# hydradarpa/kalman-hydra

Measured on AMD Instinct MI355X. Metric: frames/sec (Brox flow + EKF update) at 1024^2, higher is better.
Workload: dtype f32 (flow, renders) / f64 (EKF sums and state)

## Files before the change

### kalman-hydra_amd/csrc/ekf.hip

```cpp
#include "hm_common.h"
#include "ekf_kernels.h"
#include "dense_kernels.h"
#include "chol_flow_kernels.h"
#include "project_kernels.h"
#include "predict_kernels.h"
#include "view_kernels.h"
#include "body_kernels.h"
#include "roi_kernels.h"
#include "smooth_kernels.h"
#include <algorithm>
#include <atomic>
#include <chrono>
#include <cmath>
#include <condition_variable>
#include <cstring>
#include <functional>
#include <mutex>
#include <set>
#include <thread>
#include <utility>
#include <vector>

struct Helper {
    std::thread th;
// ... 21 lines not shown
        }
    }
    void post(std::function<int()> f)
    {
        std::unique_lock<std::mutex> lk(m);
        if (!th.joinable()) th = std::thread([this] { run(); });
        job = std::move(f);
        posted = busy = true;
        cv.notify_all();
    }
    int wait()
    {
        std::unique_lock<std::mutex> lk(m);
        cv.wait(lk, [&] { return !busy; });
        const int r = rc;
        rc = HM_OK;
        return r;
    }
    void stop()
    {
        {
            std::unique_lock<std::mutex> lk(m);
            cv.wait(lk, [&] { return !busy; });
            quit = true;
            cv.notify_all();
        }
        if (th.joinable()) th.join();
    }
};

struct hm_ctx {
    int device, W, H, N, T, E, njobs;
    HmOwner own{1};
    Helper helper;
    bool helper_used = false;
    int tail_async = 1;
    double eps_Z, eps_J, eps_M;
    hipStream_t stream;
    int *d_tri, *d_star_off, *d_star_tri, *d_edges;
    int *d_nb_off = nullptr, *d_nb_u = nullptr, *d_nb_e = nullptr;
    float *d_uv;
    uint8_t *d_tex;
    std::vector<int> edges;
    uint8_t *d_yim, *d_ym;
    float *d_yfx, *d_yfy, *d_yfxm, *d_yfym;
    bool obs_owned = true;
    const uint8_t *o_yim, *o_ym;
    const float *o_yfx, *o_yfy;
    bool have_tex, have_obs, have_ref;
    Targets ref, P, Q;
    TriSetup *d_setup, *d_cfgs;
    int4 *d_ubox;
    int *d_tlist = nullptr, *d_tcount = nullptr;
    unsigned *d_tmask = nullptr;
    double *d_X, *d_out, *d_partial;
    uint8_t *d_im8, *d_m8;
    std::vector<double> X0;
    double *d_HTH;
    double *d_H, *d_Hz, *d_Hzc, *d_invW0, *d_Af[2], *d_T[2], *d_step, *d_Wtmp, *d_X0, *d_Xn, *d_Wprior, *d_gain, *d_Awork, *d_Lt[2];
    std::vector<double> upd_X0;
    int upd_last = -1, upd_prev = -1;
    double *d_Wres;
    double *pin;
    size_t pin_n;
    int *pin_scratch;
    std::vector<double> resv, tailv;
    int result_delay = 0;
    bool tail_pending = false;
    bool tail_valid = false;
    long long tail_ticket = 0;
    hipStream_t tail_stream = nullptr;
    const uint8_t *armed_mask = nullptr;
    std::vector<int> sp_h_off, sp_h_bar, sp_h_other;
    std::vector<double> sp_h_blk;
    std::vector<int32_t> sp_bars_cached;
    std::vector<int> tri;
    DPool pool;
    int *d_area;
    int *d_sp_off, *d_sp_bar, *d_sp_other;
    double *d_sp_blk;
    bool upd_open;
    bool prefactored;
    std::vector<double> h_partial;
    int red_blocks = 512;
    double *d_tpart = nullptr;
    std::vector<double> h_tpart;
    int ntiles = 0;
    int render_rows = RI_H;
    bool last_err_valid = false;
    double last_err[4] = {0, 0, 0, 0};
    std::vector<double> last_err_X;
    long long run_ticket;
    int vsplit = 5, esplit;
    bool pn_armed = false;
    void *pn_worker = nullptr;
    std::vector<int32_t> pn_bars;
    std::vector<double> pn_l0;
    double pn_par[4] = {0, 0, 0, 0};
    int pn_maxiter = 0;
    bool pq_armed = false;
    double pq_eps_F = 0.0;
    bool pq_valid = false;
    std::vector<double> pq_X, pq_l0;
    std::vector<int32_t> pq_bars;
    double pq_par[4] = {0, 0, 0, 0};
    hipStream_t stream3 = nullptr;
// ... 269 lines not shown
    h->eps_Z = eps_Z; h->eps_J = eps_J; h->eps_M = eps_M;
    h->tri.assign(tri, tri + (size_t)3 * T);
    for (const auto &e : eset) { h->edges.push_back(e.first); h->edges.push_back(e.second); }
    h->E = (int)eset.size();
    h->njobs = N + h->E;
    h->esplit = 2 * h->E > 1024 ? 1 : 2;
    const size_t n = (size_t)W * H;
    int rc = HM_OK;
    auto step = [&](int r) { if (rc == HM_OK) rc = r; };
    step(upload(h->own, &h->d_tri, tri, (size_t)3 * T));
    step(upload(h->own, &h->d_uv, uv, (size_t)2 * N));
    step(upload(h->own, &h->d_star_off, off.data(), off.size()));
    step(upload(h->own, &h->d_star_tri, flat.data(), flat.size()));
    step(upload(h->own, &h->d_edges, h->edges.data(), h->edges.size()));
    {
        std::vector<std::vector<std::pair<int, int>>> nb(N);
        for (int e = 0; e < h->E; e++) {
            const int a = h->edges[2 * e], b = h->edges[2 * e + 1];
            nb[a].push_back(std::make_pair(b, e));
            nb[b].push_back(std::make_pair(a, e));
        }
        std::vector<int> noff(N + 1, 0), nu, ne;
        for (int v = 0; v < N; v++) {
            std::sort(nb[v].begin(), nb[v].end());
            noff[v + 1] = noff[v] + (int)nb[v].size();
            for (const auto &q : nb[v]) { nu.push_back(q.first); ne.push_back(q.second); }
            if (rc == HM_OK && 4 * ((int)nb[v].size() + 1) > PREP_MAX_ENTRIES) {
                hm_set_error("hm_ctx_create: vertex %d has %d neighbours, limit %d", v, (int)nb[v].size(), PREP_MAX_ENTRIES / 4 - 1);
                rc = HM_ERR_ARG;
            }
        }
        step(upload(h->own, &h->d_nb_off, noff.data(), noff.size()));
        step(upload(h->own, &h->d_nb_u, nu.data(), nu.size()));
        step(upload(h->own, &h->d_nb_e, ne.data(), ne.size()));
    }
    hipError_t e = hipSuccess;
    auto dev = [&](auto **p, size_t bytes) { if (e == hipSuccess) e = h->own.alloc(p, bytes); };
    if (rc == HM_OK) {
        const char *pe = getenv("HYDRA_MI_EKF_PRIORITY");
        e = h->own.stream(&h->stream, !(pe && atoi(pe) == 0));
        dev(&h->d_tex, n);
        dev(&h->d_yim, n);
        dev(&h->d_ym, n);
        dev(&h->d_yfx, n * sizeof(float));
        dev(&h->d_yfy, n * sizeof(float));
        dev(&h->d_yfxm, n * sizeof(float));
        dev(&h->d_yfym, n * sizeof(float));
        dev(&h->d_setup, (size_t)T * sizeof(TriSetup));
        dev(&h->d_cfgs, (size_t)N * MEAS_NCFG * (EKF_MAX_STAR + 1) * sizeof(TriSetup));
        dev(&h->d_ubox, (size_t)N * UBOX_STRIDE * sizeof(int4));
        dev(&h->d_tmask, (size_t)N * TMASK_STRIDE * sizeof(unsigned));
        dev(&h->d_tlist, (size_t)N * TMASK_STRIDE * sizeof(int));
        dev(&h->d_tcount, (size_t)N * sizeof(int));
        dev(&h->d_X, (size_t)4 * N * sizeof(double));
        dev(&h->d_out, (size_t)h->njobs * MEAS_VSPLIT_MAX * MEAS_OUT * sizeof(double));
        dev(&h->d_partial, (size_t)h->red_blocks * 4 * sizeof(double));
        h->ntiles = hm_cdiv(W, RI_W) * hm_cdiv(H, 8);
        dev(&h->d_tpart, (size_t)h->ntiles * RI_NV * sizeof(double));
        dev(&h->d_im8, n);
        dev(&h->d_m8, n);
        const size_t n4 = (size_t)4 * N, nn = n4 * n4 * sizeof(double);
        dev(&h->d_H, nn);
        dev(&h->d_HTH, nn);
        if (e == hipSuccess) e = hipMemsetAsync(h->d_HTH, 0, nn, h->stream);
        dev(&h->d_invW0, nn);
        const size_t nn_aug = (size_t)(hm_cdiv((int)n4, DNB) * DNB + DNB) * n4 * sizeof(double);
        dev(&h->d_Af[0], nn_aug);
        dev(&h->d_Af[1], nn_aug);
        dev(&h->d_Awork, nn_aug);
        const size_t ld_bytes = (size_t)hm_cdiv((int)n4, DNB) * DNB * DNB * sizeof(double);
        dev(&h->d_T[0], nn);
        dev(&h->d_T[1], nn);
        dev(&h->d_step, n4 * sizeof(double));
        dev(&h->d_Lt[0], ld_bytes);
        dev(&h->d_Lt[1], ld_bytes);
        dev(&h->d_Wtmp, nn);
        dev(&h->d_flowP, 3 * ld_bytes);
        dev(&h->d_flowctl, 4 * sizeof(unsigned));
        if (e == hipSuccess) e = hipMemsetAsync(h->d_flowctl, 0, 4 * sizeof(unsigned), h->stream);
        dev(&h->d_Hz, n4 * sizeof(double));
        dev(&h->d_Hzc, n4 * 4 * sizeof(double));
        dev(&h->d_Wprior, nn);
        dev(&h->d_gain, n4 * 3 * sizeof(double));
        h->pin_n = 2 * (n4 + RES_HEAD + n4 * 4 + n4 * 3) + 2;
        if (e == hipSuccess) e = h->own.host_alloc(&h->pin, h->pin_n * sizeof(double), hipHostMallocCoherent);
        if (e == hipSuccess) memset(h->pin, 0, h->pin_n * sizeof(double));
        h->pin_scratch = (int *)(h->pin + h->pin_n - 2);
        h->resv.assign(n4 + RES_HEAD, 0.0);
        h->tailv.assign(n4 * 7, 0.0);
        dev(&h->d_X0, n4 * sizeof(double));
        dev(&h->pool.hdr, (size_t)4 * N * sizeof(int));
        dev(&h->pool.overflow, sizeof(int));
        dev(&h->d_area, (size_t)N * sizeof(int));
        h->pool.area = h->d_area;
        if (e == hipSuccess) e = pool_alloc(h, (long long)8 * W * H);
        dev(&h->d_Xn, n4 * sizeof(double));
        for (Targets *t : {&h->ref, &h->P, &h->Q})
            if (e == hipSuccess) e = alloc_targets(h->own, *t, n);
    }
    if (e != hipSuccess) {
        hm_set_error("hm_ctx_create: device allocation failed: %s", hipGetErrorString(e));
        step(HM_ERR_HIP);
    }
    if (rc != HM_OK) {
        ctx_free(h);
        return rc;
// ... 453 lines not shown
    rc = render_ids(h, h->X0.data(), h->ref, h->d_ids[0], true);
    if (rc == HM_OK) rc = render_ids(h, Xp.data(), h->P, h->d_ids[1], false);
    if (rc == HM_OK) rc = render_ids(h, Xq.data(), h->Q, h->d_ids[2], false);
    if (rc) return rc;
    MultiArgs a = {h->ref, h->P, h->Q, h->d_ids[0], h->d_ids[1], h->d_ids[2], obs_of(h, 0), h->W, h->d_lbox, h->d_lout};
    hipLaunchKernelGGL(k_j_multi, dim3(n_labels), dim3(RED_NT), 0, h->stream, a);
    HM_HIP(hipGetLastError());
    h->h_lout.resize((size_t)n_labels * 5);
    HM_HIP(hipMemcpyAsync(h->h_lout.data(), h->d_lout, (size_t)n_labels * 5 * sizeof(double), hipMemcpyDeviceToHost, h->stream));
    HM_HIP(hipStreamSynchronize(h->stream));
    for (int l = 0; l < n_labels; l++) {
        const double *s = h->h_lout.data() + 5 * l;
        const double c[4] = {s[0] / h->eps_Z, s[1] / h->eps_J, s[2] / h->eps_J, s[3] / h->eps_M};
        hsum[l] = ((c[0] + c[1]) + c[2]) + c[3];
        nz[l] = s[4];
        if (hcomp) for (int k = 0; k < 4; k++) hcomp[4 * l + k] = c[k];
    }
    return HM_OK;
}

extern "C" int hm_error(hm_ctx_t h, const double *X, int masked, double err[4], float *fx, float *fy)
{
    HM_ARG(h && X && err, "hm_error: NULL argument");
    HM_JOIN(h);
    NEED_TEX(h, "hm_error");
    NEED_OBS(h, "hm_error");
    HM_HIP(hipSetDevice(h->device));
    HM_HIP(hipMemcpyAsync(h->d_X, X, (size_t)4 * h->N * sizeof(double), hipMemcpyHostToDevice, h->stream));
    int rc = render_iter(h, h->d_X, h->P, true, masked, false, 2.0);
    if (rc) return rc;
    const int n = h->W * h->H;
    if (fx) HM_HIP(hipMemcpyAsync(fx, h->P.fx, (size_t)n * sizeof(float), hipMemcpyDeviceToHost, h->stream));
    if (fy) HM_HIP(hipMemcpyAsync(fy, h->P.fy, (size_t)n * sizeof(float), hipMemcpyDeviceToHost, h->stream));
    HM_HIP(hipMemcpyAsync(h->h_tpart.data(), h->d_tpart, (size_t)render_strips(h) * RI_NV * sizeof(double), hipMemcpyDeviceToHost, h->stream));
    HM_HIP(stream_wait(h->stream));
    double s6[RI_NV];
    hm_tile_partial_sums(h->h_tpart.data(), render_strips(h), s6);
    for (int k = 0; k < 4; k++) err[k] = s6[k];
    return HM_OK;
}

static int measure_dev(hm_ctx *h, const double *dX, bool ref_ready, double deltaX, int masked, bool regions_ready = false,
                       bool scatter = true)
{
    if (!ref_ready) {
        int rc = render_iter(h, dX, h->ref, false, masked, !regions_ready, deltaX);
        if (rc) return rc;
        regions_ready = true;
    }
    MeasureArgs a;
    measure_args(h, dX, deltaX, masked, a);
    if (!regions_ready) hipLaunchKernelGGL(k_star_regions, dim3(h->N), dim3(REGION_NT), 0, h->stream, a, h->d_area);
    hipLaunchKernelGGL(k_measure_vertex, dim3(h->N, h->vsplit), dim3(MEAS_NT), 0, h->stream, a,
                       (const TriSetup *)h->d_cfgs, (const int4 *)h->d_ubox, (const unsigned *)h->d_tmask);
    if (h->E > 0) hipLaunchKernelGGL(k_measure_edge, dim3(h->E, h->esplit), dim3(MEAS_NT), 0, h->stream, a);
    if (scatter) {
        ScatterArgs s = {h->d_out, h->d_edges, h->N, h->E, h->vsplit, h->esplit, h->eps_Z, h->eps_J, h->eps_M, deltaX, h->d_HTH, h->d_Hz, h->d_Hzc};
        hipLaunchKernelGGL(k_hth_scatter, dim3(hm_cdiv(h->njobs, 4)), dim3(256), 0, h->stream, s);
    }
    HM_HIP(hipGetLastError());
    return HM_OK;
}

static void measure_args(hm_ctx *h, const double *dX, double deltaX, int masked, MeasureArgs &a)
{
    a.m = Mesh{h->W, h->H, h->N, h->T, h->d_tri, h->d_uv, h->d_tex};
    a.topo = StarTopo{h->d_star_off, h->d_star_tri, h->d_edges, h->E};
    a.ref = h->ref;
    a.obs = obs_of(h, masked);
    a.X = dX;
    a.delta = deltaX;
    a.out = h->d_out;
    a.pool = h->pool;
    a.vsplit = h->vsplit;
    a.esplit = h->esplit;
    a.iZ = 1.0 / h->eps_Z; a.iJ = 1.0 / h->eps_J; a.iM = 1.0 / h->eps_M;
    a.cfgs = h->d_cfgs;
    a.ubox = h->d_ubox;
    a.tmask = h->d_tmask;
    a.tlist = h->d_tlist;
    a.tcount = h->d_tcount;
    a.tmask_stride = TMASK_STRIDE;
}

static int measure_on_device(hm_ctx *h, const double *X, double deltaX, int masked, bool scatter = true)
{
    HM_HIP(hipMemcpyAsync(h->d_X, X, (size_t)4 * h->N * sizeof(double), hipMemcpyHostToDevice, h->stream));
    h->X0.assign(X, X + 4 * h->N);
    h->have_ref = true;
    return measure_dev(h, h->d_X, false, deltaX, masked, false, scatter);
}

extern "C" int hm_measure(hm_ctx_t h, const double *X, double deltaX, int masked, double *Hz, double *Hzc, double *HTH)
{
    HM_ARG(h && X && Hz && HTH, "hm_measure: NULL argument");
    HM_JOIN(h);
    HM_ARG(deltaX > 0, "hm_measure: deltaX must be positive");
    NEED_TEX(h, "hm_measure");
    NEED_OBS(h, "hm_measure");
    HM_HIP(hipSetDevice(h->device));
    const size_t n4 = (size_t)4 * h->N;
    int *ovf = h->pin_scratch;
    for (int attempt = 0;; attempt++) {
        int rc = measure_on_device(h, X, deltaX, masked);
        if (rc) return rc;
        *ovf = 0;
        HM_HIP(hipMemcpyAsync(ovf, h->pool.overflow, sizeof(int), hipMemcpyDeviceToHost, h->stream));
        HM_HIP(hipStreamSynchronize(h->stream));
        if (!*ovf) break;
        if (attempt) { hm_set_error("hm_measure: the star regions do not fit the difference-image pool"); return HM_ERR_STATE; }
        rc = pool_grow(h, "hm_measure");
        if (rc) return rc;
    }
    HM_HIP(hipMemcpyAsync(Hz, h->d_Hz, n4 * sizeof(double), hipMemcpyDeviceToHost, h->stream));
    if (Hzc) HM_HIP(hipMemcpyAsync(Hzc, h->d_Hzc, n4 * 4 * sizeof(double), hipMemcpyDeviceToHost, h->stream));
    HM_HIP(hipMemcpyAsync(HTH, h->d_HTH, n4 * n4 * sizeof(double), hipMemcpyDeviceToHost, h->stream));
    HM_HIP(hipStreamSynchronize(h->stream));
    return HM_OK;
}

static int aug_rows(int n) { return hm_cdiv(n, DNB) * DNB + DNB; }

static void chol_factor(hm_ctx *h, double *A, double *L, double *Lt, double *T, double *M, int n, bool with_rhs,
                        bool first_done = false, hipStream_t st = nullptr)
{
    if (!st) st = h->stream;
    const int nb = hm_cdiv(n, DNB);
    const int nrows = with_rhs ? aug_rows(n) : n;
    const int nbr = hm_cdiv(nrows, DNB);
    if (h->chol_flow) {
        FlowArgs a = {A, L, Lt, T, h->d_flowP, n, nrows, nb, nbr, h->d_flowctl, h->flow_stall};
        if (!first_done) hipLaunchKernelGGL(k_flow_fill, dim3(nrows + FLOW_FILL_WGS), dim3(256), 0, st, a);
        hipLaunchKernelGGL(k_chol_flow, dim3(h->flow_wgs), dim3(FLOW_NT), 0, st, a);
        return;
    }
// ... 2122 lines not shown
```

### kalman-hydra_amd/csrc/ekf_kernels.h

```cpp
#pragma once
#include <hip/hip_runtime.h>
#include <stdint.h>

#define EKF_SUB 256
#define EKF_MAX_STAR 24
#define EKF_TILE 16
#define EKF_MAX_TRI 4096

struct TriSetup {
    double ea[3], eb[3], ec[3];
    double ecb[3];
    int cmin, cmax, rmin, rmax;
    int tl[3];
    float inv;
    int i0, i1, i2;
    float ux[3], uy[3], ax[3], ay[3];
};

__device__ __forceinline__ void d_tri_attr(TriSetup &s, const float *__restrict__ uv, const double *__restrict__ X, int N)
{
    const int id[3] = {s.i0, s.i1, s.i2};
    for (int k = 0; k < 3; k++) {
        s.ux[k] = uv[2 * id[k]];
        s.uy[k] = uv[2 * id[k] + 1];
// ... 310 lines not shown
    d_block_reduce<4, RED_NT>(s, s_red, a.out + 4 * lab);
}

__global__ __launch_bounds__(RED_NT) void k_j_multi(MultiArgs a)
{
    __shared__ double s_red[(RED_NT / 64) * 5];
    const int lab = blockIdx.x;
    const int4 b = a.box[lab];
    double s[5] = {0, 0, 0, 0, 0};
    const int bw = b.y - b.x + 1, bh = b.w - b.z + 1;
    const int npx = (bw > 0 && bh > 0) ? bw * bh : 0;
    for (int k = threadIdx.x; k < npx; k += RED_NT) {
        const int i = (b.z + k / bw) * a.W + b.x + k % bw;
        const bool m = a.ref.cnt[i] > 0, mp = a.p.cnt[i] > 0, mq = a.q.cnt[i] > 0;
        const int face = m ? a.idr[i] : (mp ? a.idp[i] : (mq ? a.idq[i] : 65535));
        if (face != lab || face >= 65535) continue;
        const int rim = a.ref.acc[i] > 255 ? 255 : a.ref.acc[i];
        const int pim = a.p.acc[i] > 255 ? 255 : a.p.acc[i], qim = a.q.acc[i] > 255 ? 255 : a.q.acc[i];
        const int rm = m ? 255 : 0, pm = mp ? 255 : 0, qm = mq ? 255 : 0;
        s[0] += ((double)(pim - rim) / 255.0) * ((double)(qim - rim) / 255.0);
        s[1] += (double)(a.p.fx[i] - a.ref.fx[i]) * (double)(a.q.fx[i] - a.ref.fx[i]);
        s[2] += (double)(a.p.fy[i] - a.ref.fy[i]) * (double)(a.q.fy[i] - a.ref.fy[i]);
        s[3] += ((double)(pm - rm) / 255.0) * ((double)(qm - rm) / 255.0);
        s[4] += 1.0;
    }
    d_block_reduce<5, RED_NT>(s, s_red, a.out + 5 * lab);
}

struct StarTopo {
    const int *star_off;
    const int *star_tri;
    const int *edges;
    int E;
};

struct StarVal {
    int acc, cnt;
    float fx, fy;
};
struct StarTex {
    int t0, t1;
};
__device__ __forceinline__ int d_star_texels(const uint8_t *__restrict__ tex, const StarTex &q)
{
    const int a = tex[q.t0 < 0 ? 0 : q.t0], b = tex[q.t1 < 0 ? 0 : q.t1];
    return (q.t0 < 0 ? 0 : a) + (q.t1 < 0 ? 0 : b);
}

struct StarVel {
    float fxp, fxm, fyp, fym;
};

template <bool VEL>
__device__ __forceinline__ StarVal d_star_eval(const TriSetup *__restrict__ cfg, unsigned mask, int c, int r,
                                               const Mesh &m, int v, float vxp, float vxm, float nvyp, float nvym,
                                               StarVel &vel, StarTex &q)
{
    StarVal s = {0, 0, 0.0f, 0.0f};
    q.t0 = -1; q.t1 = -1;
    if (VEL) { vel.fxp = 0.0f; vel.fxm = 0.0f; vel.fyp = 0.0f; vel.fym = 0.0f; }
    const double dc = (double)c, dr = (double)r;
    auto add = [&](const TriSetup &t, double e1, double e2) {
        float l1, l2;
        d_tri_bary2(t, e1, e2, l1, l2);
        const int at = d_texel_at(t, l1, l2, m.W, m.H);
        if (s.cnt == 0) q.t0 = at;
        else if (s.cnt == 1) q.t1 = at;
        else s.acc += m.tex[at];
        const float a0 = t.ax[0], a1 = t.ax[1], a2 = t.ax[2];
        const float b0 = t.ay[0], b1 = t.ay[1], b2 = t.ay[2];
        s.fx = s.fx + d_lerp(a0, a1, a2, l1, l2);
        s.fy = s.fy + d_lerp(b0, b1, b2, l1, l2);
        s.cnt++;
        if (VEL) {
            const bool v0 = t.i0 == v, v1 = t.i1 == v, v2 = t.i2 == v;
            vel.fxp = vel.fxp + d_lerp(v0 ? vxp : a0, v1 ? vxp : a1, v2 ? vxp : a2, l1, l2);
            vel.fxm = vel.fxm + d_lerp(v0 ? vxm : a0, v1 ? vxm : a1, v2 ? vxm : a2, l1, l2);
            vel.fyp = vel.fyp + d_lerp(v0 ? nvyp : b0, v1 ? nvyp : b1, v2 ? nvyp : b2, l1, l2);
            vel.fym = vel.fym + d_lerp(v0 ? nvym : b0, v1 ? nvym : b1, v2 ? nvym : b2, l1, l2);
        }
    };
    for (unsigned mm = mask; mm != 0; mm &= mm - 1) {
        const TriSetup &t = cfg[__builtin_ctz(mm)];
        double e1, e2;
        if (d_tri_cover2(t, dc, dr, e1, e2)) add(t, e1, e2);
    }
    return s;
}

__device__ __forceinline__ int d_i255(double x) { return (int)rint(x * 255.0); }

struct Diff {
    double im, m;
    float fx, fy;
};

__device__ __forceinline__ void d_fill_k255(double *tab, int nthreads)
{
    for (int i = threadIdx.x; i < 511; i += nthreads) tab[i] = (double)(i - 255) / 255.0;
}
__device__ __forceinline__ double d_q255(const double *k255, int x)
{
    return (x >= -255 && x <= 255) ? k255[x] : (double)x / 255.0;
}

__device__ __forceinline__ Diff d_diff(const double *k255, int racc, int rcnt, float rfx, float rfy, const StarVal &sref,
                                       const StarVal &sp)
{
    int rim = racc > 255 ? 255 : racc;
    int pacc = racc - sref.acc + sp.acc;
    int pim = pacc > 255 ? 255 : pacc;
    int rm = rcnt > 0 ? 255 : 0;
    int pm = (rcnt - sref.cnt + sp.cnt) > 0 ? 255 : 0;
    Diff d;
    d.im = k255[pim - rim];
    d.m = (double)((pm - rm) / 255);
    float pfx = (rfx - sref.fx) + sp.fx;
    float pfy = (rfy - sref.fy) + sp.fy;
    d.fx = pfx - rfx;
    d.fy = pfy - rfy;
    return d;
}

__device__ inline void d_star_setup_one(TriSetup &out, int t, const Mesh &m, const double *X, int v, double dx, double dy)
{
    int v0 = m.tri[3 * t], v1 = m.tri[3 * t + 1], v2 = m.tri[3 * t + 2];
    double px[3] = {X[2 * v0], X[2 * v1], X[2 * v2]}, py[3] = {X[2 * v0 + 1], X[2 * v1 + 1], X[2 * v2 + 1]};
    int vs[3] = {v0, v1, v2};
    for (int q = 0; q < 3; q++)
        if (vs[q] == v) { px[q] += dx; py[q] += dy; }
    d_tri_setup(out, v0, v1, v2, d_snap(px[0]), d_snap(py[0]), d_snap(px[1]), d_snap(py[1]), d_snap(px[2]),
                d_snap(py[2]), m.W, m.H);
    d_tri_attr(out, m.uv, X, m.N);
}
__device__ inline void d_star_setup_pad(TriSetup &e)
{
    e.cmin = 1; e.cmax = 0; e.rmin = 1; e.rmax = 0;
    for (int k = 0; k < 3; k++) { e.ea[k] = 0.0; e.eb[k] = 0.0; e.ec[k] = -1.0; e.ecb[k] = -1.0; e.tl[k] = 0; }
}
__device__ inline void d_star_setups(TriSetup *dst, int ns, const int *tris, const Mesh &m, const double *X, int v,
                                     double dx, double dy, int lane, int stride)
{
    for (int k = lane; k < ns; k += stride) d_star_setup_one(dst[k], tris[k], m, X, v, dx, dy);
    if ((ns & 1) && lane == 0) d_star_setup_pad(dst[ns]);
}

#define POOL_EMPTY 0x7FFF
struct DPool {
    int *hdr;
    int *live;
    const int *area;
    short2 *xi, *yi;
    float *xfx, *xfy, *yfx, *yfy, *vxfx, *vyfy;
    long long cap;
    int *overflow;
};

__device__ __forceinline__ void d_park_empty(const DPool &P, long long pp)
{
    P.xi[pp] = make_short2(POOL_EMPTY, 0); P.yi[pp] = make_short2(0, 0);
    P.xfx[pp] = 0.0f; P.xfy[pp] = 0.0f; P.yfx[pp] = 0.0f; P.yfy[pp] = 0.0f;
    P.vxfx[pp] = 0.0f; P.vyfy[pp] = 0.0f;
}

struct MeasureArgs {
    Mesh m;
    StarTopo topo;
    Targets ref;
    Obs obs;
    const double *X;
    double delta;
    double *out;
    DPool pool;
    int vsplit;
    int esplit;
    double iZ, iJ, iM;
    TriSetup *cfgs;
    int4 *ubox;
    unsigned *tmask;
    int *tlist, *tcount;
    int tmask_stride;
};

#define MEAS_NT 256
#define MEAS_OUT 40
#define MEAS_VSPLIT_MAX 16
enum {
    A_X = 0, A_Y = 4, A_VX = 8, A_VY = 9,
    A_XX = 10, A_XY = 11, A_YY = 12,
    A_XVX = 13, A_YVX = 14,
    A_XVY = 15, A_YVY = 16,
    A_VXVX = 17, A_VYVY = 18,
    A_NV = 19
};
enum {
    B_XX = 0, B_XY = 1, B_YX = 2, B_YY = 3,
    B_XVX = 4, B_YVX = 5, B_VXX = 6, B_VXY = 7, B_VXVX = 8,
    B_XVY = 9, B_YVY = 10, B_VYX = 11, B_VYY = 12, B_VYVY = 13,
    B_NV = 14
};

#define MEAS_NCFG 5
#define UBOX_STRIDE (EKF_MAX_STAR + 4)
#define TMASK_STRIDE 1024

__device__ inline void d_vertex_cfgs(TriSetup (*cfg)[EKF_MAX_STAR + 1], int nsv, const int *trv, const Mesh &m,
                                     const double *X, int v, double d, int nthreads)
{
    const int wv = threadIdx.x >> 6, lane = threadIdx.x & 63, nw = nthreads >> 6;
    const double dxs[MEAS_NCFG] = {0, d, -d, 0, 0}, dys[MEAS_NCFG] = {0, 0, 0, d, -d};
    for (int c = wv; c < MEAS_NCFG; c += nw) d_star_setups(cfg[c], nsv, trv, m, X, v, dxs[c], dys[c], lane, 64);
}

#define REGION_NT (64 * MEAS_NCFG)
struct RegionShared {
    int4 tbox[MEAS_NCFG][EKF_MAX_STAR + 1];
    double ea[MEAS_NCFG][EKF_MAX_STAR + 1][3], eb[MEAS_NCFG][EKF_MAX_STAR + 1][3], ecb[MEAS_NCFG][EKF_MAX_STAR + 1][3];
    int box[MEAS_NCFG][4];
    int reg[4];
    int wsum[8];
};
template <int NT>
__device__ inline void d_star_regions(const MeasureArgs &a, int *__restrict__ area, int v, RegionShared &sh)
{
    const Mesh &m = a.m;
    const int nsv = a.topo.star_off[v + 1] - a.topo.star_off[v];
    const int *trv = a.topo.star_tri + a.topo.star_off[v];
    const int wv = threadIdx.x >> 6, lane = threadIdx.x & 63;
    constexpr int NW = NT / 64;
    const double d = a.delta;
    const double dxs[MEAS_NCFG] = {0, d, -d, 0, 0}, dys[MEAS_NCFG] = {0, 0, 0, d, -d};
    for (int cf = wv; cf < MEAS_NCFG; cf += NW) {
        TriSetup *dst = a.cfgs + ((size_t)v * MEAS_NCFG + cf) * (EKF_MAX_STAR + 1);
        if (lane < nsv) {
            TriSetup su;
            d_star_setup_one(su, trv[lane], m, a.X, v, dxs[cf], dys[cf]);
            dst[lane] = su;
            sh.tbox[cf][lane] = make_int4(su.cmin, su.cmax, su.rmin, su.rmax);
            for (int k = 0; k < 3; k++) { sh.ea[cf][lane][k] = su.ea[k]; sh.eb[cf][lane][k] = su.eb[k]; sh.ecb[cf][lane][k] = su.ecb[k]; }
        }
        if ((nsv & 1) && lane == 0) {
            TriSetup pad;
            d_star_setup_pad(pad);
            pad.inv = 0.0f; pad.i0 = pad.i1 = pad.i2 = 0;
            for (int k = 0; k < 3; k++) { pad.ux[k] = pad.uy[k] = pad.ax[k] = pad.ay[k] = 0.0f; }
            dst[nsv] = pad;
        }
    }
    __syncthreads();
    if (wv == 0 && lane < UBOX_STRIDE) {
        int4 u = make_int4(1, 0, 1, 0);
        if (lane < nsv)
            for (int cfg = 0; cfg < MEAS_NCFG; cfg++) {
                const int4 s = sh.tbox[cfg][lane];
                if (s.x > s.y) continue;
                if (u.x > u.y) u = s;
                else u = make_int4(min(u.x, s.x), max(u.y, s.y), min(u.z, s.z), max(u.w, s.w));
            }
        a.ubox[(size_t)v * UBOX_STRIDE + lane] = u;
    }
    for (int cf = wv; cf < MEAS_NCFG; cf += NW) {
        int c0 = m.W, c1 = -1, r0 = m.H, r1 = -1;
        if (lane < nsv) {
            const int4 s = sh.tbox[cf][lane];
            if (s.x <= s.y) { c0 = s.x; c1 = s.y; r0 = s.z; r1 = s.w; }
        }
        for (int o = 16; o > 0; o >>= 1) {
            c0 = min(c0, __shfl_down(c0, o, 64)); c1 = max(c1, __shfl_down(c1, o, 64));
            r0 = min(r0, __shfl_down(r0, o, 64)); r1 = max(r1, __shfl_down(r1, o, 64));
        }
        if (lane == 0) { sh.box[cf][0] = c0; sh.box[cf][1] = c1; sh.box[cf][2] = r0; sh.box[cf][3] = r1; }
    }
    __syncthreads();
    if (threadIdx.x == 0) {
        int c0 = m.W, c1 = -1, r0 = m.H, r1 = -1;
        for (int cfg = 0; cfg < MEAS_NCFG; cfg++) {
            c0 = min(c0, sh.box[cfg][0]); c1 = max(c1, sh.box[cfg][1]);
            r0 = min(r0, sh.box[cfg][2]); r1 = max(r1, sh.box[cfg][3]);
        }
        if (c1 >= c0) { c0 &= ~7; r0 &= ~7; }
        const int rw = c1 >= c0 ? (c1 - c0 + 8) & ~7 : 0, rh = (c1 >= c0 && r1 >= r0) ? (r1 - r0 + 8) & ~7 : 0;
        a.pool.hdr[4 * v] = c0; a.pool.hdr[4 * v + 1] = r0; a.pool.hdr[4 * v + 2] = rw; a.pool.hdr[4 * v + 3] = rh;
        area[v] = rw * rh;
        sh.reg[0] = c0; sh.reg[1] = r0; sh.reg[2] = rw; sh.reg[3] = rh;
    }
    __syncthreads();
    const int ntx = sh.reg[2] >> 3, ntiles = ntx * (sh.reg[3] >> 3);
    if (ntiles > a.tmask_stride) {
        if (threadIdx.x == 0) a.tcount[v] = -1;
        return;
    }
    int listed = 0;
    for (int t0 = 0; t0 < ntiles; t0 += NT) {
        const int t = t0 + threadIdx.x;
        unsigned word = 0;
        if (t < ntiles) {
            const int tc0 = sh.reg[0] + 8 * (t % ntx), tr0 = sh.reg[1] + 8 * (t / ntx);
            const double xa = (double)tc0, xb = (double)min(tc0 + 7, m.W - 1), ya = (double)tr0, yb = (double)min(tr0 + 7, m.H - 1);
#pragma unroll 1
            for (int k = 0; k < nsv; k++) {
                bool reach = false;
#pragma unroll 1
                for (int cf = 0; cf < MEAS_NCFG && !reach; cf++) {
                    const int4 b = sh.tbox[cf][k];
                    if ((b.x > b.y) | (b.y < tc0) | (b.x > tc0 + 7) | (b.w < tr0) | (b.z > tr0 + 7)) continue;
                    bool in = true;
#pragma unroll 1
                    for (int e = 0; e < 3; e++) {
                        const double A = sh.ea[cf][k][e], B = sh.eb[cf][k][e], C = sh.ecb[cf][k][e];
                        const double e00 = fma(A, xa, fma(B, ya, C)), e10 = fma(A, xb, fma(B, ya, C));
                        const double e01 = fma(A, xa, fma(B, yb, C)), e11 = fma(A, xb, fma(B, yb, C));
                        in &= (e00 > 0.0) | (e10 > 0.0) | (e01 > 0.0) | (e11 > 0.0);
                    }
                    reach = in;
                }
                if (reach) word |= 1u << k;
            }
            a.tmask[(size_t)v * a.tmask_stride + t] = word;
        }
        const unsigned long long bal = __ballot(word != 0);
        __syncthreads();
        if (lane == 0) sh.wsum[wv] = __popcll(bal);
        __syncthreads();
        int before = listed;
        for (int w = 0; w < wv; w++) before += sh.wsum[w];
        if (word != 0) a.tlist[(size_t)v * a.tmask_stride + before + __popcll(bal & ((1ull << lane) - 1ull))] = t;
        for (int w = 0; w < NW; w++) listed += sh.wsum[w];
    }
    if (threadIdx.x == 0) a.tcount[v] = listed;
}

__global__ __launch_bounds__(REGION_NT) void k_star_regions(MeasureArgs a, int *__restrict__ area)
{
    __shared__ RegionShared sh;
    d_star_regions<REGION_NT>(a, area, blockIdx.x, sh);
}

template <int NT>
__device__ inline void d_region_sums(const int *__restrict__ area, int N, int v, int w, long long &bv, long long &bw,
                                     long long &tot, long long *s )
{
    long long a = 0, b = 0, c = 0;
    for (int i = threadIdx.x; i < N; i += NT) {
        const long long x = area[i];
        c += x;
        if (i < v) a += x;
        if (i < w) b += x;
    }
    for (int o = 32; o > 0; o >>= 1) {
        a += __shfl_down(a, o, 64); b += __shfl_down(b, o, 64); c += __shfl_down(c, o, 64);
    }
    const int lane = threadIdx.x & 63, wv = threadIdx.x >> 6;
    if (lane == 0) { s[wv * 3] = a; s[wv * 3 + 1] = b; s[wv * 3 + 2] = c; }
    __syncthreads();
    bv = 0; bw = 0; tot = 0;
    for (int k = 0; k < NT / 64; k++) { bv += s[k * 3]; bw += s[k * 3 + 1]; tot += s[k * 3 + 2]; }
}

#ifndef MEAS_OCC
#define MEAS_OCC 4
#endif
__global__ __launch_bounds__(MEAS_NT, MEAS_OCC) void k_measure_vertex(MeasureArgs a, const TriSetup *__restrict__ cfgs,
                                                                const int4 *__restrict__ ubox, const unsigned *__restrict__ tmask)
{
    __shared__ double s_red[(MEAS_NT / 64) * MEAS_OUT];
    __shared__ double s_k255[511];
    const double *k255 = s_k255 + 255;
    d_fill_k255(s_k255, MEAS_NT);
    const Mesh &m = a.m;
    const int N = m.N, W = m.W;
    const int v = blockIdx.x, job = v;
    const double *X = a.X;
    const double d = a.delta;
    const int nsv = a.topo.star_off[v + 1] - a.topo.star_off[v];
    const TriSetup *__restrict__ s_cfg[MEAS_NCFG];
#pragma unroll
    for (int c = 0; c < MEAS_NCFG; c++) s_cfg[c] = cfgs + ((size_t)v * MEAS_NCFG + c) * (EKF_MAX_STAR + 1);
    __syncthreads();
    const int c0 = a.pool.hdr[4 * v], r0 = a.pool.hdr[4 * v + 1], rw = a.pool.hdr[4 * v + 2], rh = a.pool.hdr[4 * v + 3];
    __shared__ long long s_sum[(MEAS_NT / 64) * 3];
    long long base, unused, total;
    d_region_sums<MEAS_NT>(a.pool.area, N, v, 0, base, unused, total, s_sum);
    const bool park = total <= a.pool.cap;
    if (v == 0 && blockIdx.y == 0 && threadIdx.x == 0) *a.pool.overflow = park ? 0 : 1;
    double acc[A_NV];
#pragma unroll
    for (int k = 0; k < A_NV; k++) acc[k] = 0.0;
    const int wave = __builtin_amdgcn_readfirstlane(threadIdx.x >> 6);
    const int lx = threadIdx.x & 7, ly = (threadIdx.x & 63) >> 3;
    const int ntx = (rw + 7) >> 3, ntiles = ntx * ((rh + 7) >> 3);
    const int nwaves = (MEAS_NT / 64) * gridDim.y;
    const int listed = a.tcount[v];
    const int nwalk = listed >= 0 ? listed : ntiles;
    for (int j = blockIdx.y * (MEAS_NT / 64) + wave; j < nwalk; j += nwaves) {
        const int tile = listed >= 0 ? a.tlist[(size_t)v * a.tmask_stride + j] : j;
        const int tr0 = r0 + 8 * (tile / ntx), tc0 = c0 + 8 * (tile % ntx);
        const int r = tr0 + ly, c = tc0 + lx;
        unsigned mask = 0;
        if (listed >= 0) {
            mask = tmask[(size_t)v * a.tmask_stride + tile];
        } else {
            for (int k = 0; k < nsv; k++) {
                const int4 b = ubox[(size_t)v * UBOX_STRIDE + k];
                if (!((b.y < tc0) | (b.x > tc0 + 7) | (b.w < tr0) | (b.z > tr0 + 7))) mask |= 1u << k;
            }
        }
        const long long pp = base + (long long)tile * 64 + (threadIdx.x & 63);
        if (c >= W || r >= m.H) {
            if (park) d_park_empty(a.pool, pp);
            continue;
        }
        const int p = r * W + c;
        const int racc = a.ref.acc[p], rcnt = a.ref.cnt[p];
        const float rfx = a.ref.fx[p], rfy = a.ref.fy[p];
        StarVel vel, none;
        StarTex q0, q1, q2, q3, q4;
        StarVal sref = d_star_eval<true>(s_cfg[0], mask, c, r, m, v, (float)(X[2 * N + 2 * v] + d),
                                         (float)(X[2 * N + 2 * v] - d), (float)(-(X[2 * N + 2 * v + 1] + d)),
                                         (float)(-(X[2 * N + 2 * v + 1] - d)), vel, q0);
        StarVal sxp = d_star_eval<false>(s_cfg[1], mask, c, r, m, v, 0, 0, 0, 0, none, q1);
        StarVal sxm = d_star_eval<false>(s_cfg[2], mask, c, r, m, v, 0, 0, 0, 0, none, q2);
        StarVal syp = d_star_eval<false>(s_cfg[3], mask, c, r, m, v, 0, 0, 0, 0, none, q3);
        StarVal sym = d_star_eval<false>(s_cfg[4], mask, c, r, m, v, 0, 0, 0, 0, none, q4);
        {
            const int e0 = d_star_texels(m.tex, q0), e1 = d_star_texels(m.tex, q1), e2 = d_star_texels(m.tex, q2);
            const int e3 = d_star_texels(m.tex, q3), e4 = d_star_texels(m.tex, q4);
            sref.acc += e0; sxp.acc += e1; sxm.acc += e2; syp.acc += e3; sym.acc += e4;
        }
        const bool covered = sref.cnt + sxp.cnt + sxm.cnt + syp.cnt + sym.cnt != 0;
        const bool tile_live = __any(covered);
        if (park && (threadIdx.x & 63) == __builtin_ctzll(__builtin_amdgcn_read_exec()))
            a.pool.live[base / 64 + tile] = tile_live ? 1 : 0;
        if (!covered) {
            if (park) d_park_empty(a.pool, pp);
            continue;
        }
        const StarVal svxp = {sref.acc, sref.cnt, vel.fxp, sref.fy}, svxm = {sref.acc, sref.cnt, vel.fxm, sref.fy};
        const StarVal svyp = {sref.acc, sref.cnt, sref.fx, vel.fyp}, svym = {sref.acc, sref.cnt, sref.fx, vel.fym};
        const Diff dxp = d_diff(k255, racc, rcnt, rfx, rfy, sref, sxp), dxm = d_diff(k255, racc, rcnt, rfx, rfy, sref, sxm);
        const Diff dyp = d_diff(k255, racc, rcnt, rfx, rfy, sref, syp), dym = d_diff(k255, racc, rcnt, rfx, rfy, sref, sym);
        const Diff dvxp = d_diff(k255, racc, rcnt, rfx, rfy, sref, svxp), dvxm = d_diff(k255, racc, rcnt, rfx, rfy, sref, svxm);
        const Diff dvyp = d_diff(k255, racc, rcnt, rfx, rfy, sref, svyp), dvym = d_diff(k255, racc, rcnt, rfx, rfy, sref, svym);
        const int rim = racc > 255 ? 255 : racc, rm = rcnt > 0 ? 255 : 0;
        const double z = k255[(int)a.obs.yim[p] - rim];
        const double zm = d_q255(k255, 255 * (int)a.obs.ym[p] - rm);
        const double zfx = (double)(a.obs.yfx[p] - rfx), zfy = (double)(a.obs.yfy[p] + rfy);
        {
            acc[A_X + 0] = fma(dxp.im - dxm.im, z, acc[A_X + 0]); acc[A_X + 1] = fma((double)dxp.fx - (double)dxm.fx, zfx, acc[A_X + 1]);
            acc[A_X + 2] = fma((double)dxp.fy - (double)dxm.fy, zfy, acc[A_X + 2]); acc[A_X + 3] = fma(dxp.m - dxm.m, zm, acc[A_X + 3]);
            acc[A_Y + 0] = fma(dyp.im - dym.im, z, acc[A_Y + 0]); acc[A_Y + 1] = fma((double)dyp.fx - (double)dym.fx, zfx, acc[A_Y + 1]);
            acc[A_Y + 2] = fma((double)dyp.fy - (double)dym.fy, zfy, acc[A_Y + 2]); acc[A_Y + 3] = fma(dyp.m - dym.m, zm, acc[A_Y + 3]);
            acc[A_VX] = fma((double)dvxp.fx - (double)dvxm.fx, zfx, acc[A_VX]);
            acc[A_VY] = fma((double)dvyp.fy - (double)dvym.fy, zfy, acc[A_VY]);
        }
        {
            const double xi = dxp.im, xf = (double)dxp.fx, xg = (double)dxp.fy, xm = dxp.m;
            const double yi = dyp.im, yf = (double)dyp.fx, yg = (double)dyp.fy, ym = dyp.m;
            const double wxi = xi * a.iZ, wxf = xf * a.iJ, wxg = xg * a.iJ, wxm = xm * a.iM;
            acc[A_XX] = fma(wxm, xm, fma(wxg, xg, fma(wxf, xf, fma(wxi, xi, acc[A_XX]))));
            acc[A_XY] = fma(wxm, ym, fma(wxg, yg, fma(wxf, yf, fma(wxi, yi, acc[A_XY]))));
            acc[A_YY] = fma(ym * a.iM, ym, fma(yg * a.iJ, yg, fma(yf * a.iJ, yf, fma(yi * a.iZ, yi, acc[A_YY]))));
            const double vf = (double)dvxp.fx, vg = (double)dvyp.fy;
            acc[A_XVX] = fma(xf, vf, acc[A_XVX]); acc[A_YVX] = fma(yf, vf, acc[A_YVX]);
            acc[A_XVY] = fma(xg, vg, acc[A_XVY]); acc[A_YVY] = fma(yg, vg, acc[A_YVY]);
            acc[A_VXVX] = fma(vf, vf, acc[A_VXVX]); acc[A_VYVY] = fma(vg, vg, acc[A_VYVY]);
        }
        if (park) {
            a.pool.xi[pp] = make_short2((short)d_i255(dxp.im), (short)d_i255(dxp.m));
            a.pool.yi[pp] = make_short2((short)d_i255(dyp.im), (short)d_i255(dyp.m));
            a.pool.xfx[pp] = dxp.fx; a.pool.xfy[pp] = dxp.fy; a.pool.yfx[pp] = dyp.fx; a.pool.yfy[pp] = dyp.fy;
            a.pool.vxfx[pp] = dvxp.fx; a.pool.vyfy[pp] = dvyp.fy;
        }
    }
    if (park && listed >= 0)
        for (int t = blockIdx.y * MEAS_NT + threadIdx.x; t < ntiles; t += MEAS_NT * gridDim.y)
            if (tmask[(size_t)v * a.tmask_stride + t] == 0) a.pool.live[base / 64 + t] = 0;
// ... 388 lines not shown
```

Baseline: 335.0.

## Share opposite-edge function across perturbed star configs in vertex measure

Restructures the per-pixel star evaluation so that the five perturbed configurations are walked together per triangle rather than in five separate passes. The edge function opposite the perturbed vertex, which is identical across configs, is computed once and reused. Which edge can be shared is detected per triangle in the region kernel and stored as two bitmasks. This cuts the double-precision FMAs and the TriSetup reads in the hot measure kernel, at the cost of more live registers and an extra small buffer and setup pass.

After: 329.9. 1.5% lower.

```diff
diff --git a/kalman-hydra_amd/csrc/ekf.hip b/kalman-hydra_amd/csrc/ekf.hip
--- a/kalman-hydra_amd/csrc/ekf.hip
+++ b/kalman-hydra_amd/csrc/ekf.hip
@@ -97,6 +97,7 @@
     TriSetup *d_setup, *d_cfgs;
     int4 *d_ubox;
     int *d_tlist = nullptr, *d_tcount = nullptr;
+    unsigned *d_tshare = nullptr;
     unsigned *d_tmask = nullptr;
     double *d_X, *d_out, *d_partial;
     uint8_t *d_im8, *d_m8;
@@ -472,6 +473,7 @@
         dev(&h->d_tmask, (size_t)N * TMASK_STRIDE * sizeof(unsigned));
         dev(&h->d_tlist, (size_t)N * TMASK_STRIDE * sizeof(int));
         dev(&h->d_tcount, (size_t)N * sizeof(int));
+        dev(&h->d_tshare, (size_t)N * 2 * sizeof(unsigned));
         dev(&h->d_X, (size_t)4 * N * sizeof(double));
         dev(&h->d_out, (size_t)h->njobs * MEAS_VSPLIT_MAX * MEAS_OUT * sizeof(double));
         dev(&h->d_partial, (size_t)h->red_blocks * 4 * sizeof(double));
@@ -1031,7 +1033,8 @@
     measure_args(h, dX, deltaX, masked, a);
     if (!regions_ready) hipLaunchKernelGGL(k_star_regions, dim3(h->N), dim3(REGION_NT), 0, h->stream, a, h->d_area);
     hipLaunchKernelGGL(k_measure_vertex, dim3(h->N, h->vsplit), dim3(MEAS_NT), 0, h->stream, a,
-                       (const TriSetup *)h->d_cfgs, (const int4 *)h->d_ubox, (const unsigned *)h->d_tmask);
+                       (const TriSetup *)h->d_cfgs, (const int4 *)h->d_ubox, (const unsigned *)h->d_tmask,
+                       (const unsigned *)h->d_tshare);
     if (h->E > 0) hipLaunchKernelGGL(k_measure_edge, dim3(h->E, h->esplit), dim3(MEAS_NT), 0, h->stream, a);
     if (scatter) {
         ScatterArgs s = {h->d_out, h->d_edges, h->N, h->E, h->vsplit, h->esplit, h->eps_Z, h->eps_J, h->eps_M, deltaX, h->d_HTH, h->d_Hz, h->d_Hzc};
@@ -1060,6 +1063,7 @@
     a.tlist = h->d_tlist;
     a.tcount = h->d_tcount;
     a.tmask_stride = TMASK_STRIDE;
+    a.tshare = h->d_tshare;
 }
 
 static int measure_on_device(hm_ctx *h, const double *X, double deltaX, int masked, bool scatter = true)
diff --git a/kalman-hydra_amd/csrc/ekf_kernels.h b/kalman-hydra_amd/csrc/ekf_kernels.h
--- a/kalman-hydra_amd/csrc/ekf_kernels.h
+++ b/kalman-hydra_amd/csrc/ekf_kernels.h
@@ -386,40 +386,78 @@
 };
 
 template <bool VEL>
-__device__ __forceinline__ StarVal d_star_eval(const TriSetup *__restrict__ cfg, unsigned mask, int c, int r,
-                                               const Mesh &m, int v, float vxp, float vxm, float nvyp, float nvym,
-                                               StarVel &vel, StarTex &q)
-{
-    StarVal s = {0, 0, 0.0f, 0.0f};
-    q.t0 = -1; q.t1 = -1;
-    if (VEL) { vel.fxp = 0.0f; vel.fxm = 0.0f; vel.fyp = 0.0f; vel.fym = 0.0f; }
+__device__ __forceinline__ void d_star_add(StarVal &s, StarTex &q, StarVel &vel, const TriSetup &t, double e1, double e2,
+                                           const Mesh &m, int v, float vxp, float vxm, float nvyp, float nvym)
+{
+    float l1, l2;
+    d_tri_bary2(t, e1, e2, l1, l2);
+    const int at = d_texel_at(t, l1, l2, m.W, m.H);
+    if (s.cnt == 0) q.t0 = at;
+    else if (s.cnt == 1) q.t1 = at;
+    else s.acc += m.tex[at];
+    const float a0 = t.ax[0], a1 = t.ax[1], a2 = t.ax[2];
+    const float b0 = t.ay[0], b1 = t.ay[1], b2 = t.ay[2];
+    s.fx = s.fx + d_lerp(a0, a1, a2, l1, l2);
+    s.fy = s.fy + d_lerp(b0, b1, b2, l1, l2);
+    s.cnt++;
+    if (VEL) {
+        const bool v0 = t.i0 == v, v1 = t.i1 == v, v2 = t.i2 == v;
+        vel.fxp = vel.fxp + d_lerp(v0 ? vxp : a0, v1 ? vxp : a1, v2 ? vxp : a2, l1, l2);
+        vel.fxm = vel.fxm + d_lerp(v0 ? vxm : a0, v1 ? vxm : a1, v2 ? vxm : a2, l1, l2);
+        vel.fyp = vel.fyp + d_lerp(v0 ? nvyp : b0, v1 ? nvyp : b1, v2 ? nvyp : b2, l1, l2);
+        vel.fym = vel.fym + d_lerp(v0 ? nvym : b0, v1 ? nvym : b1, v2 ? nvym : b2, l1, l2);
+    }
+}
+template <int OPP>
+__device__ __forceinline__ bool d_tri_cover_opp(const TriSetup &t, double dc, double dr, double eo, bool po, double &e1, double &e2)
+{
+    const double e0 = OPP == 0 ? eo : fma(t.ea[0], dc, fma(t.eb[0], dr, t.ecb[0]));
+    e1 = OPP == 1 ? eo : fma(t.ea[1], dc, fma(t.eb[1], dr, t.ecb[1]));
+    e2 = OPP == 2 ? eo : fma(t.ea[2], dc, fma(t.eb[2], dr, t.ecb[2]));
+    const bool p0 = OPP == 0 ? po : e0 > 0.0, p1 = OPP == 1 ? po : e1 > 0.0, p2 = OPP == 2 ? po : e2 > 0.0;
+    return p0 & p1 & p2;
+}
+__device__ __forceinline__ void d_star_tri(const TriSetup *__restrict__ const (&cfg)[5], int k, int code, double dc, double dr, const Mesh &m,
+                                           int v, float vxp, float vxm, float nvyp, float nvym, StarVal (&s)[5],
+                                           StarTex (&q)[5], StarVel &vel)
+{
+    double eo, e1, e2;
+    bool po;
+    {
+        const TriSetup &t = cfg[0][k];
+        const double e0 = fma(t.ea[0], dc, fma(t.eb[0], dr, t.ecb[0]));
+        e1 = fma(t.ea[1], dc, fma(t.eb[1], dr, t.ecb[1]));
+        e2 = fma(t.ea[2], dc, fma(t.eb[2], dr, t.ecb[2]));
+        eo = code == 2 ? e1 : (code == 3 ? e2 : e0);
+        po = eo > 0.0;
+        if ((e0 > 0.0) & (e1 > 0.0) & (e2 > 0.0)) d_star_add<true>(s[0], q[0], vel, t, e1, e2, m, v, vxp, vxm, nvyp, nvym);
+    }
+#pragma unroll
+    for (int c = 1; c < 5; c++) {
+        const TriSetup &t = cfg[c][k];
+        bool in;
+        switch (code) {
+        case 1: in = d_tri_cover_opp<0>(t, dc, dr, eo, po, e1, e2); asm volatile("" ::: "memory"); break;
+        case 2: in = d_tri_cover_opp<1>(t, dc, dr, eo, po, e1, e2); asm volatile("" ::: "memory"); break;
+        case 3: in = d_tri_cover_opp<2>(t, dc, dr, eo, po, e1, e2); asm volatile("" ::: "memory"); break;
+        default: in = d_tri_cover_opp<-1>(t, dc, dr, eo, po, e1, e2); asm volatile("" ::: "memory"); break;
+        }
+        if (in) d_star_add<false>(s[c], q[c], vel, t, e1, e2, m, v, 0, 0, 0, 0);
+    }
+}
+__device__ __forceinline__ void d_star_eval5(const TriSetup *__restrict__ const (&cfg)[5], unsigned mask, unsigned share_lo,
+                                             unsigned share_hi, int c, int r, const Mesh &m, int v, float vxp, float vxm,
+                                             float nvyp, float nvym, StarVal (&s)[5], StarTex (&q)[5], StarVel &vel)
+{
+#pragma unroll
+    for (int i = 0; i < 5; i++) { s[i] = StarVal{0, 0, 0.0f, 0.0f}; q[i].t0 = -1; q[i].t1 = -1; }
+    vel.fxp = 0.0f; vel.fxm = 0.0f; vel.fyp = 0.0f; vel.fym = 0.0f;
     const double dc = (double)c, dr = (double)r;
-    auto add = [&](const TriSetup &t, double e1, double e2) {
-        float l1, l2;
-        d_tri_bary2(t, e1, e2, l1, l2);
-        const int at = d_texel_at(t, l1, l2, m.W, m.H);
-        if (s.cnt == 0) q.t0 = at;
-        else if (s.cnt == 1) q.t1 = at;
-        else s.acc += m.tex[at];
-        const float a0 = t.ax[0], a1 = t.ax[1], a2 = t.ax[2];
-        const float b0 = t.ay[0], b1 = t.ay[1], b2 = t.ay[2];
-        s.fx = s.fx + d_lerp(a0, a1, a2, l1, l2);
-        s.fy = s.fy + d_lerp(b0, b1, b2, l1, l2);
-        s.cnt++;
-        if (VEL) {
-            const bool v0 = t.i0 == v, v1 = t.i1 == v, v2 = t.i2 == v;
-            vel.fxp = vel.fxp + d_lerp(v0 ? vxp : a0, v1 ? vxp : a1, v2 ? vxp : a2, l1, l2);
-            vel.fxm = vel.fxm + d_lerp(v0 ? vxm : a0, v1 ? vxm : a1, v2 ? vxm : a2, l1, l2);
-            vel.fyp = vel.fyp + d_lerp(v0 ? nvyp : b0, v1 ? nvyp : b1, v2 ? nvyp : b2, l1, l2);
-            vel.fym = vel.fym + d_lerp(v0 ? nvym : b0, v1 ? nvym : b1, v2 ? nvym : b2, l1, l2);
-        }
-    };
     for (unsigned mm = mask; mm != 0; mm &= mm - 1) {
-        const TriSetup &t = cfg[__builtin_ctz(mm)];
-        double e1, e2;
-        if (d_tri_cover2(t, dc, dr, e1, e2)) add(t, e1, e2);
-    }
-    return s;
+        const int k = __builtin_ctz(mm);
+        const int code = __builtin_amdgcn_readfirstlane((int)(((share_lo >> k) & 1u) | (((share_hi >> k) & 1u) << 1)));
+        d_star_tri(cfg, k, code, dc, dr, m, v, vxp, vxm, nvyp, nvym, s, q, vel);
+    }
 }
 
 __device__ __forceinline__ int d_i255(double x) { return (int)rint(x * 255.0); }
@@ -514,6 +552,7 @@
     unsigned *tmask;
     int *tlist, *tcount;
     int tmask_stride;
+    unsigned *tshare;
 };
 
 #define MEAS_NT 256
@@ -550,6 +589,7 @@
 struct RegionShared {
     int4 tbox[MEAS_NCFG][EKF_MAX_STAR + 1];
     double ea[MEAS_NCFG][EKF_MAX_STAR + 1][3], eb[MEAS_NCFG][EKF_MAX_STAR + 1][3], ecb[MEAS_NCFG][EKF_MAX_STAR + 1][3];
+    int opp[MEAS_NCFG][EKF_MAX_STAR + 1];
     int box[MEAS_NCFG][4];
     int reg[4];
     int wsum[8];
@@ -572,6 +612,7 @@
             dst[lane] = su;
             sh.tbox[cf][lane] = make_int4(su.cmin, su.cmax, su.rmin, su.rmax);
             for (int k = 0; k < 3; k++) { sh.ea[cf][lane][k] = su.ea[k]; sh.eb[cf][lane][k] = su.eb[k]; sh.ecb[cf][lane][k] = su.ecb[k]; }
+            sh.opp[cf][lane] = su.i0 == v ? 0 : (su.i1 == v ? 1 : 2);
         }
         if ((nsv & 1) && lane == 0) {
             TriSetup pad;
@@ -592,6 +633,19 @@
                 else u = make_int4(min(u.x, s.x), max(u.y, s.y), min(u.z, s.z), max(u.w, s.w));
             }
         a.ubox[(size_t)v * UBOX_STRIDE + lane] = u;
+    }
+    if (wv == 0) {
+        int code = 0;
+        if (lane < nsv) {
+            const int o = sh.opp[0][lane];
+            bool same = true;
+            for (int cfg = 1; cfg < MEAS_NCFG; cfg++)
+                same = same && sh.opp[cfg][lane] == o && sh.ea[cfg][lane][o] == sh.ea[0][lane][o] &&
+                       sh.eb[cfg][lane][o] == sh.eb[0][lane][o] && sh.ecb[cfg][lane][o] == sh.ecb[0][lane][o];
+            if (same) code = o + 1;
+        }
+        const unsigned lo = (unsigned)__ballot(code & 1), hi = (unsigned)__ballot(code & 2);
+        if (lane == 0) { a.tshare[2 * v] = lo; a.tshare[2 * v + 1] = hi; }
     }
     for (int cf = wv; cf < MEAS_NCFG; cf += NW) {
         int c0 = m.W, c1 = -1, r0 = m.H, r1 = -1;
@@ -695,7 +749,8 @@
 #define MEAS_OCC 4
 #endif
 __global__ __launch_bounds__(MEAS_NT, MEAS_OCC) void k_measure_vertex(MeasureArgs a, const TriSetup *__restrict__ cfgs,
-                                                                const int4 *__restrict__ ubox, const unsigned *__restrict__ tmask)
+                                                                const int4 *__restrict__ ubox, const unsigned *__restrict__ tmask,
+                                                                const unsigned *__restrict__ tshare)
 {
     __shared__ double s_red[(MEAS_NT / 64) * MEAS_OUT];
     __shared__ double s_k255[511];
@@ -725,6 +780,7 @@
     const int ntx = (rw + 7) >> 3, ntiles = ntx * ((rh + 7) >> 3);
     const int nwaves = (MEAS_NT / 64) * gridDim.y;
     const int listed = a.tcount[v];
+    const unsigned share_lo = tshare[2 * v], share_hi = tshare[2 * v + 1];
     const int nwalk = listed >= 0 ? listed : ntiles;
     for (int j = blockIdx.y * (MEAS_NT / 64) + wave; j < nwalk; j += nwaves) {
         const int tile = listed >= 0 ? a.tlist[(size_t)v * a.tmask_stride + j] : j;
@@ -745,17 +801,15 @@
             continue;
         }
         const int p = r * W + c;
+        StarVel vel;
+        StarVal sv[5];
+        StarTex qv[5];
+        d_star_eval5(s_cfg, mask, share_lo, share_hi, c, r, m, v, (float)(X[2 * N + 2 * v] + d), (float)(X[2 * N + 2 * v] - d),
+                     (float)(-(X[2 * N + 2 * v + 1] + d)), (float)(-(X[2 * N + 2 * v + 1] - d)), sv, qv, vel);
+        StarVal &sref = sv[0], &sxp = sv[1], &sxm = sv[2], &syp = sv[3], &sym = sv[4];
+        const StarTex &q0 = qv[0], &q1 = qv[1], &q2 = qv[2], &q3 = qv[3], &q4 = qv[4];
         const int racc = a.ref.acc[p], rcnt = a.ref.cnt[p];
         const float rfx = a.ref.fx[p], rfy = a.ref.fy[p];
-        StarVel vel, none;
-        StarTex q0, q1, q2, q3, q4;
-        StarVal sref = d_star_eval<true>(s_cfg[0], mask, c, r, m, v, (float)(X[2 * N + 2 * v] + d),
-                                         (float)(X[2 * N + 2 * v] - d), (float)(-(X[2 * N + 2 * v + 1] + d)),
-                                         (float)(-(X[2 * N + 2 * v + 1] - d)), vel, q0);
-        StarVal sxp = d_star_eval<false>(s_cfg[1], mask, c, r, m, v, 0, 0, 0, 0, none, q1);
-        StarVal sxm = d_star_eval<false>(s_cfg[2], mask, c, r, m, v, 0, 0, 0, 0, none, q2);
-        StarVal syp = d_star_eval<false>(s_cfg[3], mask, c, r, m, v, 0, 0, 0, 0, none, q3);
-        StarVal sym = d_star_eval<false>(s_cfg[4], mask, c, r, m, v, 0, 0, 0, 0, none, q4);
         {
             const int e0 = d_star_texels(m.tex, q0), e1 = d_star_texels(m.tex, q1), e2 = d_star_texels(m.tex, q2);
             const int e3 = d_star_texels(m.tex, q3), e4 = d_star_texels(m.tex, q4);
```
